# Thealexbarney/VGAudio

Hardware: NVIDIA H100
Metric: GC-ADPCM encode Msamples/sec (batch) (higher is better)
Workload: dtype int32

## Files before the change

vgaudio_b200/csrc/abi_gcadpcm.cu:

```cuda
#include <climits>

#include "abi.cuh"

using namespace vgb;

namespace {

struct GcLayout {
    int32_t n_channels = 0;
    std::vector<int64_t> pcm_off, adpcm_off, rec_off;
    std::vector<int32_t> n_samples, enc_count;
    std::vector<int16_t> hist;
    int64_t pcm_total = 0;
    int64_t adpcm_total = 0;
    int64_t rec_total = 0;
    int32_t max_frames = 0;
    int64_t total_frames = 0;
};

struct GcWorkspace {
    size_t off_pcm_off, off_adpcm_off, off_rec_off, off_n_samples, off_enc_count, off_hist, off_records, off_mask;
    size_t off_trace, off_used_start, off_stats;
    size_t off_status;
    size_t table_bytes;
    size_t total;
};

GcWorkspace carve(int64_t rec_total_frames, int32_t n_channels)
{
    GcWorkspace w{};
    size_t o = 0;
    auto take = [&](size_t bytes) { size_t at = o; o = align_up(o + bytes, 256); return at; };
    const size_t n = (size_t)(n_channels > 0 ? n_channels : 1);
    w.off_pcm_off = take(n * 8);
    w.off_adpcm_off = take(n * 8);
    w.off_rec_off = take(n * 8);
    w.off_n_samples = take(n * 4);
    w.off_enc_count = take(n * 4);
    w.off_hist = take(n * 4);
    w.table_bytes = o;
    w.off_records = take((size_t)rec_total_frames * sizeof(double2));
    w.off_mask = take((size_t)(rec_total_frames / 32 + 1) * 4);
    w.off_trace = take((size_t)rec_total_frames * 4);
    w.off_used_start = take(n * kGcMaxSegments * 4);
    w.off_stats = take(kGcStatWords * 8);
    w.off_status = take(16);
    w.total = o;
    return w;
}

int64_t padded_rec_bound(int64_t total_frames, int32_t n_channels) { return total_frames + 32ll * n_channels + 32; }

GcChannelTable table_view(void *ws, const GcWorkspace &w, int32_t n_channels)
{
    char *b = static_cast<char *>(ws);
    GcChannelTable t;
    t.pcm_off = reinterpret_cast<const int64_t *>(b + w.off_pcm_off);
    t.adpcm_off = reinterpret_cast<const int64_t *>(b + w.off_adpcm_off);
    t.rec_off = reinterpret_cast<const int64_t *>(b + w.off_rec_off);
    t.n_samples = reinterpret_cast<const int32_t *>(b + w.off_n_samples);
    t.enc_count = reinterpret_cast<const int32_t *>(b + w.off_enc_count);
    t.hist = reinterpret_cast<int16_t *>(b + w.off_hist);
    t.status = reinterpret_cast<int32_t *>(b + w.off_status);
    t.n_channels = n_channels;
    return t;
}

GcSegArgs seg_view(void *ws, const GcWorkspace &w, int32_t seg_count)
{
    char *b = static_cast<char *>(ws);
    GcSegArgs a;
    a.trace = reinterpret_cast<uint32_t *>(b + w.off_trace);
    a.used_start = reinterpret_cast<uint32_t *>(b + w.off_used_start);
    a.stats = reinterpret_cast<unsigned long long *>(b + w.off_stats);
    a.seg_count = seg_count;
    a.min_seg_frames = 0;
    return a;
}

int32_t upload_tables(const GcLayout &lay, const GcWorkspace &w, void *ws, cudaStream_t stream)
{
    std::vector<char> blob(w.table_bytes, 0);
    const size_t n = (size_t)lay.n_channels;
    if (n) {
        memcpy(blob.data() + w.off_pcm_off, lay.pcm_off.data(), n * 8);
        memcpy(blob.data() + w.off_adpcm_off, lay.adpcm_off.data(), n * 8);
        memcpy(blob.data() + w.off_rec_off, lay.rec_off.data(), n * 8);
        memcpy(blob.data() + w.off_n_samples, lay.n_samples.data(), n * 4);
        memcpy(blob.data() + w.off_enc_count, lay.enc_count.data(), n * 4);
        memcpy(blob.data() + w.off_hist, lay.hist.data(), n * 4);
    }
    CUDA_TRY(cudaMemcpyAsync(ws, blob.data(), w.table_bytes, cudaMemcpyHostToDevice, stream));
    return VGB_OK;
}

void layout_records(GcLayout &lay)
{
    lay.rec_off.resize(lay.n_channels);
    int64_t rec = 0;
    for (int c = 0; c < lay.n_channels; c++) {
        const int32_t frames = div_round_up(lay.n_samples[c], kGcFrameSamples);
        lay.rec_off[c] = rec;
        rec += (int64_t)align_up((size_t)frames, 32);
        if (frames > lay.max_frames) lay.max_frames = frames;
        lay.total_frames += div_round_up(lay.enc_count[c], kGcFrameSamples);
    }
    lay.rec_total = rec + 32;
}

int32_t layout_common(GcLayout &lay, const int32_t *n_samples, const vgb_gc_params *params, int32_t n_channels,
                      bool decode)
{
    if (n_channels < 0) return fail(VGB_E_ARG, "n_channels is negative (%d)", n_channels);
    if (n_channels > 0 && !n_samples) return fail(VGB_E_ARG, "n_samples is NULL");
    lay.n_channels = n_channels;
    lay.n_samples.resize(n_channels);
    lay.enc_count.resize(n_channels);
    lay.hist.assign((size_t)n_channels * 2, 0);
    for (int c = 0; c < n_channels; c++) {
        const int32_t n = n_samples[c];
        if (n < 0) return fail(VGB_E_ARG, "channel %d: negative sample count %d", c, n);
        int32_t enc = n;
        if (params) {
            if (!decode && params[c].sample_count != -1) {
                enc = params[c].sample_count;
                if (enc < 0 || enc > n)
                    return fail(VGB_E_ARG, "channel %d: sample_count %d outside the %d available samples", c, enc, n);
            }
            lay.hist[2 * c] = params[c].history1;
            lay.hist[2 * c + 1] = params[c].history2;
        }
        lay.n_samples[c] = n;
        lay.enc_count[c] = enc;
    }
    layout_records(lay);
    return VGB_OK;
}

void layout_pack_offsets(GcLayout &lay)
{
    lay.pcm_off.resize(lay.n_channels);
    lay.adpcm_off.resize(lay.n_channels);
    int64_t ps = 0, ab = 0;
    for (int c = 0; c < lay.n_channels; c++) {
        lay.pcm_off[c] = ps;
        lay.adpcm_off[c] = ab;
        ps += (int64_t)align_up((size_t)lay.n_samples[c], 8);
        ab += (int64_t)align_up((size_t)gc_sample_count_to_byte_count(lay.n_samples[c]), 16);
    }
    lay.pcm_total = ps + 8;
    lay.adpcm_total = ab + 16;
}

int max_encode_frames(const GcLayout &lay)
{
    int32_t m = 0;
    for (int c = 0; c < lay.n_channels; c++) m = std::max(m, div_round_up(lay.enc_count[c], kGcFrameSamples));
    return m;
}

int32_t run_gc_encode(const int16_t *d_pcm, const GcLayout &lay, const int16_t *d_coefs_in, int16_t *d_coefs_out,
                      uint8_t *d_adpcm, void *d_ws, const GcWorkspace &w, cudaStream_t stream, bool do_encode,
                      bool timed = true, bool tables_uploaded = false, cudaEvent_t after_coefs = nullptr)
{
    const bool was_timing = g_ctx.timing;
    if (!timed) g_ctx.timing = false;
    struct Restore { bool v; ~Restore() { g_ctx.timing = v; } } restore{was_timing};
    if (!tables_uploaded) VGB_TRY(upload_tables(lay, w, d_ws, stream));
    if (lay.n_channels == 0) return VGB_OK;
    GcChannelTable tab = table_view(d_ws, w, lay.n_channels);
    char *b = static_cast<char *>(d_ws);
    double2 *records = reinterpret_cast<double2 *>(b + w.off_records);
    uint32_t *mask = reinterpret_cast<uint32_t *>(b + w.off_mask);

    if (!d_coefs_in) {
        tick(0, true, stream);
        launch_gc_coef_frames(d_pcm, tab, records, mask, lay.max_frames, 0, INT_MAX, stream);
        tick(0, false, stream);
        tick(1, true, stream);
        launch_gc_coef_refine(tab, records, mask, d_coefs_out, stream);
        tick(1, false, stream);
        g_ctx.launches += (lay.max_frames > 0 ? 1 : 0) + 1;
    } else if (d_coefs_in != d_coefs_out) {
        CUDA_TRY(cudaMemcpyAsync(d_coefs_out, d_coefs_in, (size_t)lay.n_channels * 32, cudaMemcpyDeviceToDevice, stream));
    }
    if (after_coefs) CUDA_TRY(cudaEventRecord(after_coefs, stream));
    if (do_encode) {
        const int enc_frames = max_encode_frames(lay);
        int min_seg = 0;
        const int seg_count = gc_encode_pick_segments(lay.n_channels, enc_frames, &min_seg);
        GcSegArgs seg = seg_view(d_ws, w, seg_count);
        seg.min_seg_frames = min_seg;
        tick(2, true, stream);
        launch_gc_encode(d_pcm, tab, d_coefs_out, d_adpcm, lay.max_frames, 0, INT_MAX, seg, stream);
        tick(2, false, stream);
        g_ctx.launches += lay.max_frames > 0 ? (seg.seg_count > 1 ? 3 : 1) : 0;
        g_ctx.last_seg = seg;
    }
    CUDA_TRY(cudaGetLastError());
    return VGB_OK;
}

int32_t run_gc_decode(const uint8_t *d_adpcm, const GcLayout &lay, const int16_t *d_coefs, int16_t *d_pcm, void *d_ws,
                      const GcWorkspace &w, cudaStream_t stream)
{
    VGB_TRY(upload_tables(lay, w, d_ws, stream));
    if (lay.n_channels == 0) return VGB_OK;
    GcChannelTable tab = table_view(d_ws, w, lay.n_channels);
    CUDA_TRY(cudaMemsetAsync(tab.status, 0x7f, 4, stream));
    tick(3, true, stream);
    launch_gc_decode(d_adpcm, tab, d_coefs, d_pcm, lay.max_frames, 0, INT_MAX, stream);
    tick(3, false, stream);
    g_ctx.launches += lay.max_frames > 0 ? 1 : 0;
    CUDA_TRY(cudaGetLastError());
    return VGB_OK;
}


GcLayout sub_layout(const GcLayout &full, int c0, int c1)
{
    GcLayout g;
    g.n_channels = c1 - c0;
    g.pcm_off.assign(full.pcm_off.begin() + c0, full.pcm_off.begin() + c1);
    g.adpcm_off.assign(full.adpcm_off.begin() + c0, full.adpcm_off.begin() + c1);
    g.n_samples.assign(full.n_samples.begin() + c0, full.n_samples.begin() + c1);
    g.enc_count.assign(full.enc_count.begin() + c0, full.enc_count.begin() + c1);
    g.hist.assign(full.hist.begin() + 2 * c0, full.hist.begin() + 2 * c1);
    layout_records(g);
    return g;
}

int32_t host_encode_impl(const int16_t *const *pcm, const int32_t *n_samples, const vgb_gc_params *params,
                         const int16_t *coefs_in, int32_t n_channels, int16_t *coefs_out, uint8_t *const *adpcm_out,
                         vgb_progress_cb cb, void *user, bool do_encode)
{
    PinScope pins;
    GcLayout lay;
    VGB_TRY(layout_common(lay, n_samples, params, n_channels, false));
    if (n_channels == 0) return VGB_OK;
    if (!pcm) return fail(VGB_E_ARG, "pcm is NULL");
    if (!coefs_out) return fail(VGB_E_ARG, "coefs_out is NULL");
    if (do_encode && !adpcm_out) return fail(VGB_E_ARG, "adpcm_out is NULL");
    for (int c = 0; c < n_channels; c++) {
        if (!pcm[c] && lay.n_samples[c] > 0) return fail(VGB_E_ARG, "pcm[%d] is NULL", c);
        if (do_encode && !adpcm_out[c] && lay.enc_count[c] > 0) return fail(VGB_E_ARG, "adpcm_out[%d] is NULL", c);
    }
    layout_pack_offsets(lay);
    std::vector<int64_t> weight(n_channels), pcm_b(n_channels), pcm_len(n_channels), adpcm_len(n_channels);
    int64_t total = 0;
    for (int c = 0; c < n_channels; c++) {
        weight[c] = lay.n_samples[c];
        total += lay.n_samples[c];
        pcm_b[c] = lay.pcm_off[c] * 2;
        pcm_len[c] = (int64_t)lay.n_samples[c] * 2;
        adpcm_len[c] = gc_sample_count_to_byte_count(lay.enc_count[c]);
    }

    const int n_groups = pipeline_group_count(n_channels, 2 * total, 32, "VGB_ENCODE_GROUPS");
    const std::vector<int> bound = pipeline_bounds(weight, n_groups);

    std::lock_guard<std::mutex> lock(g_ctx.mu);
    VGB_TRY(ensure_ready_locked());
    std::vector<GcLayout> glay(n_groups);
    std::vector<GcWorkspace> gws(n_groups);
    std::vector<size_t> ws_at(n_groups);
    size_t ws_total = 0;
    for (int g = 0; g < n_groups; g++) {
        glay[g] = sub_layout(lay, bound[g], bound[g + 1]);
        gws[g] = carve(glay[g].rec_total, glay[g].n_channels);
        ws_at[g] = ws_total;
        ws_total += align_up(gws[g].total, 256);
    }
    VGB_TRY(g_ctx.pcm.reserve((size_t)lay.pcm_total * 2));
    VGB_TRY(g_ctx.adpcm.reserve((size_t)lay.adpcm_total));
    VGB_TRY(g_ctx.coefs.reserve((size_t)n_channels * 32 * 2));
    VGB_TRY(g_ctx.ws.reserve(ws_total));
    int16_t *d_coefs_out = static_cast<int16_t *>(g_ctx.coefs.p);
    int16_t *d_coefs_in = coefs_in ? d_coefs_out + (size_t)n_channels * 16 : nullptr;

    auto h2d = [&](int g) -> int32_t {
        const int c0 = bound[g], n = bound[g + 1] - c0;
        if (g == 0)
            for (int k = 0; k < n_groups; k++) VGB_TRY(upload_tables(glay[k], gws[k], g_ctx.ws.c() + ws_at[k], g_ctx.s_in));
        VGB_TRY(copy_units(cudaMemcpyHostToDevice, g_ctx.pcm.c(), pcm_b.data(), pcm, pcm_len.data(), c0, n, g_ctx.s_in));
        if (coefs_in && n > 0)
            CUDA_TRY(cudaMemcpyAsync(d_coefs_in + (size_t)c0 * 16, coefs_in + (size_t)c0 * 16, (size_t)n * 32,
                                     cudaMemcpyHostToDevice, g_ctx.s_in));
        return VGB_OK;
    };
    auto kern = [&](int g, cudaStream_t st, cudaEvent_t coefs_done) -> int32_t {
        const int c0 = bound[g];
        return run_gc_encode(static_cast<const int16_t *>(g_ctx.pcm.p), glay[g], d_coefs_in ? d_coefs_in + (size_t)c0 * 16 : nullptr,
                             d_coefs_out + (size_t)c0 * 16, static_cast<uint8_t *>(g_ctx.adpcm.p), g_ctx.ws.c() + ws_at[g], gws[g],
                             st, do_encode, false, true, coefs_done);
    };
    auto d2h = [&](int g) -> int32_t {
        const int c0 = bound[g], n = bound[g + 1] - c0;
        if (n > 0)
            CUDA_TRY(cudaMemcpyAsync(coefs_out + (size_t)c0 * 16, d_coefs_out + (size_t)c0 * 16, (size_t)n * 32,
                                     cudaMemcpyDeviceToHost, g_ctx.s_out));
        if (!do_encode) return VGB_OK;
        return copy_units(cudaMemcpyDeviceToHost, g_ctx.adpcm.c(), lay.adpcm_off.data(), adpcm_out, adpcm_len.data(), c0, n, g_ctx.s_out);
    };
    auto done = [&](int g) -> int32_t {
        if (cb && do_encode && glay[g].total_frames > 0) cb(user, glay[g].total_frames);
        return VGB_OK;
    };
    return run_group_pipeline(n_groups, h2d, kern, d2h, done);
}

int32_t host_encode_sharded(const int16_t *const *pcm, const int32_t *n_samples, const vgb_gc_params *params,
                            const int16_t *coefs_in, int32_t n_channels, int16_t *coefs_out, uint8_t *const *adpcm_out,
                            vgb_progress_cb cb, void *user, bool do_encode)
{
    if (!sharding_active(n_channels) || !pcm || !n_samples || !coefs_out || (do_encode && !adpcm_out))
        return host_encode_impl(pcm, n_samples, params, coefs_in, n_channels, coefs_out, adpcm_out, cb, user, do_encode);
    SharedProgress prog{cb, user, {}};
    return run_sharded(shard_units(n_channels, [&](int c) { return n_samples[c]; }, 64), [&](int, const std::vector<int> &u) -> int32_t {
        const int m = (int)u.size();
        auto s_pcm = pick_rows(pcm, u);
        auto s_n = pick_rows(n_samples, u);
        std::vector<vgb_gc_params> s_par;
        if (params) s_par = pick_rows(params, u);
        std::vector<int16_t> s_cin, s_cout((size_t)m * 16);
        if (coefs_in) s_cin = pick_rows(coefs_in, u, 16);
        std::vector<uint8_t *> s_out;
        if (do_encode) s_out = pick_rows(adpcm_out, u);
        VGB_TRY(host_encode_impl(s_pcm.data(), s_n.data(), params ? s_par.data() : nullptr, coefs_in ? s_cin.data() : nullptr, m,
                                 s_cout.data(), do_encode ? s_out.data() : nullptr, cb ? SharedProgress::relay : nullptr, &prog, do_encode));
        put_rows(coefs_out, u, s_cout, 16);
        return VGB_OK;
    });
}

}

extern "C" {

int32_t vgb_gcadpcm_sample_count_to_byte_count(int32_t n) { return gc_sample_count_to_byte_count(n); }
int32_t vgb_gcadpcm_byte_count_to_sample_count(int32_t b) { return gc_nibble_count_to_sample_count(b * 2); }
int32_t vgb_gcadpcm_sample_count_to_nibble_count(int32_t n) { return gc_sample_count_to_nibble_count(n); }
int32_t vgb_gcadpcm_nibble_count_to_sample_count(int32_t n) { return gc_nibble_count_to_sample_count(n); }
int32_t vgb_gcadpcm_sample_to_nibble(int32_t s)
{
    return kGcFrameNibbles * (s / kGcFrameSamples) + s % kGcFrameSamples + 2;
}
int32_t vgb_gcadpcm_nibble_to_sample(int32_t nib)
{
    return kGcFrameSamples * (nib / kGcFrameNibbles) + nib % kGcFrameNibbles - 2;
}

int32_t vgb_gcadpcm_coefs_batch(const int16_t *const *pcm, const int32_t *n_samples, int32_t n_channels,
                                int16_t *coefs_out)
{
    return host_encode_sharded(pcm, n_samples, nullptr, nullptr, n_channels, coefs_out, nullptr, nullptr, nullptr, false);
}

int32_t vgb_gcadpcm_encode_batch(const int16_t *const *pcm, const int32_t *n_samples, const vgb_gc_params *params,
                                 const int16_t *coefs_in, int32_t n_channels, int16_t *coefs_out,
                                 uint8_t *const *adpcm_out, vgb_progress_cb cb, void *user)
{
    return host_encode_sharded(pcm, n_samples, params, coefs_in, n_channels, coefs_out, adpcm_out, cb, user, true);
}

static int32_t gcadpcm_decode_one(const uint8_t *const *adpcm, const int32_t *n_bytes, const int16_t *coefs,
                                  const vgb_gc_params *params, int32_t n_channels, int16_t *const *pcm_out)
{
    PinScope pins;
    if (n_channels < 0) return fail(VGB_E_ARG, "n_channels is negative (%d)", n_channels);
    if (n_channels == 0) return VGB_OK;
    if (!adpcm || !n_bytes || !coefs || !pcm_out) return fail(VGB_E_ARG, "NULL argument");
    std::vector<int32_t> counts(n_channels);
    for (int c = 0; c < n_channels; c++) {
        if (n_bytes[c] < 0) return fail(VGB_E_ARG, "channel %d: negative byte count", c);
        int32_t want = (params && params[c].sample_count != -1) ? params[c].sample_count
                                                                : gc_nibble_count_to_sample_count(n_bytes[c] * 2);
        if (want < 0) return fail(VGB_E_ARG, "channel %d: negative sample count %d", c, want);
// ... 407 lines not shown
```

vgaudio_b200/csrc/common.cuh:

```cuda
#pragma once

#include <cuda_runtime.h>
#include <stdint.h>

namespace vgb {

constexpr int kGcFrameSamples = 14;
constexpr int kGcFrameBytes = 8;
constexpr int kGcFrameNibbles = 16;

__host__ __device__ __forceinline__ int32_t wadd(int32_t a, int32_t b) { return (int32_t)((uint32_t)a + (uint32_t)b); }
__host__ __device__ __forceinline__ int32_t wsub(int32_t a, int32_t b) { return (int32_t)((uint32_t)a - (uint32_t)b); }
__host__ __device__ __forceinline__ int32_t wmul(int32_t a, int32_t b) { return (int32_t)((uint32_t)a * (uint32_t)b); }

__host__ __device__ __forceinline__ int32_t clamp16(int32_t v) { return v > 32767 ? 32767 : (v < -32768 ? -32768 : v); }
__host__ __device__ __forceinline__ int32_t clamp4(int32_t v) { return v > 7 ? 7 : (v < -8 ? -8 : v); }

__host__ __device__ __forceinline__ int32_t gc_sample_count_to_nibble_count(int32_t n)
{
    int32_t whole = n / kGcFrameSamples, rest = n % kGcFrameSamples;
    return kGcFrameNibbles * whole + (rest == 0 ? 0 : rest + 2);
}
__host__ __device__ __forceinline__ int32_t gc_sample_count_to_byte_count(int32_t n)
{
    int32_t nib = gc_sample_count_to_nibble_count(n);
    return nib / 2 + (nib & 1);
}
__host__ __device__ __forceinline__ int32_t gc_nibble_count_to_sample_count(int32_t nib)
{
    int32_t whole = nib / kGcFrameNibbles, rest = nib % kGcFrameNibbles;
    return kGcFrameSamples * whole + (rest < 2 ? 0 : rest - 2);
}
__host__ __device__ __forceinline__ int32_t div_round_up(int32_t a, int32_t b) { return (int32_t)(((int64_t)a + b - 1) / b); }

struct GcChannelTable {
    const int64_t *pcm_off;
    const int64_t *adpcm_off;
    const int64_t *rec_off;
    const int32_t *n_samples;
    const int32_t *enc_count;
    int16_t *hist;
    int32_t *status;
    int32_t n_channels;
};

constexpr int kGcMinSegFrames = 4096;
constexpr int kGcMaxSegments = 256;
constexpr int kGcStatWords = 18;
struct GcSegArgs {
    uint32_t *trace;
    uint32_t *used_start;
    unsigned long long *stats;
    int32_t seg_count;
    int32_t min_seg_frames;
};

struct GcTapChannel {
    int64_t out_off;
    int32_t samples_per_entry;
    int32_t loop_start;
};

struct AdxChannel {
    int64_t pcm_off;
    int64_t adpcm_off;
    int32_t n_samples;
    int32_t frame_size, version, padding, type, filter;
    int32_t history;
    int16_t coef0, coef1;
    int64_t trace_off;
};

constexpr int kAdxMinSegFrames = 4096;
constexpr int kAdxMaxSegments = 64;
struct AdxSegArgs {
    uint32_t *trace;
    uint32_t *used_start;
    unsigned long long *stats;
    int32_t seg_count;
    int32_t min_seg_frames;
};

constexpr int32_t VGB_HCA_BITRATE_TOO_LOW = 1;
constexpr int32_t VGB_HCA_NOT_IMPLEMENTED = 2;
constexpr int32_t VGB_HCA_BIT_OVERFLOW = 3;
constexpr int32_t VGB_HCA_BAD_SYNC = 4;
constexpr int32_t VGB_HCA_BAD_INDEX = 6;
constexpr int32_t VGB_HCA_BAD_DELTA = 5;

struct HcaConfig {
    int32_t channel_count, frame_size;
    int32_t base_band_count, stereo_band_count, total_band_count, hfr_band_count, bands_per_hfr_group, hfr_group_count;
    int32_t channel_type[8];
    uint8_t ath[128];
};

struct HcaStream {
    int64_t pcm_off;
    int64_t channel_stride;
    int64_t frames_off;
    int64_t dct_off;
    int32_t sample_count, frame_count;
    int32_t inserted_samples, reserved;
    int32_t pre_zero, pre_fill, post_count, loop_start, src_count, last_chunk;
};

struct HcaTables {
    const double *window;
    const double *sin_tab[8], *cos_tab[8];
    const int32_t *shuffle;
    double mdct_scale, sqrt2;
    const double *dequantizer_scaling, *quantizer_scaling;
    const double *inv_step, *dead_zone;
    const double *intensity_bounds;
    const uint8_t *scale_to_resolution;
    const uint8_t *quantized_max_bits;
    const uint8_t (*quantize_bits)[16];
    const uint8_t (*quantize_value)[16];
    const uint16_t *crc_table;
    const double *step_size;
    const double *intensity_ratio;
    const double *scale_conversion;
    const uint8_t (*dequantize_bits)[16];
    const int8_t (*dequantize_value)[16];
};

}
```

vgaudio_b200/csrc/gc_encode.cu:

```cuda
#include <algorithm>
#include <cstdlib>

#include "common.cuh"
#include "kernels.h"

namespace vgb {

constexpr uint32_t kFull = 0xFFFFFFFFu;
constexpr int kEncChunkFrames = 16;
constexpr int kEncChunkSamples = kEncChunkFrames * kGcFrameSamples;
constexpr int kEncWarps = 2;
constexpr int kEncWarpChannels = 4;
constexpr int kEncRowPad = 4;
#ifndef VGB_ENC_BLOCKS_PER_SM
#define VGB_ENC_BLOCKS_PER_SM 8
#endif
constexpr int kEncChainBlocksPerSm = VGB_ENC_BLOCKS_PER_SM;
constexpr uint32_t kErrSat = (1u << 27) - 1;

template <bool kGeneral>
struct GcTrial {
    uint32_t w0, w1;
    int32_t r1, r2;
    int32_t over;
    uint64_t err;
    int32_t recon[kGeneral ? 14 : 1];
};

__device__ __forceinline__ int32_t gc_quantise_exact(int32_t diff, int shift)
{
    const uint32_t a = diff < 0 ? (0u - (uint32_t)diff) : (uint32_t)diff;
    const uint32_t top = a >> 24;
    const uint32_t hs = top ? (0x80000000u >> __clz(top)) : 0u;
    const uint32_t m = (a + (1u << (shift - 1)) - 1u - hs) >> shift;
    return diff < 0 ? -(int32_t)m : (int32_t)m;
}

template <bool kGeneral>
__device__ __forceinline__ void gc_attempt_exact(const int16_t *frame, int n, int32_t h1, int32_t h2, int32_t c0,
                                              int32_t c1, int sp, GcTrial<kGeneral> &t)
{
    const int shift = sp + 11;
    const int32_t scale = (int32_t)(1u << shift);
    int32_t r1 = h1, r2 = h2, over = 0;
    uint64_t err = 0;
    uint32_t w0 = 0, w1 = 0;
#pragma unroll
    for (int s = 0; s < 14; s++) {
        if (kGeneral && s >= n) break;
        const int32_t xs = frame[s];
        const int32_t want = xs * 2048;
        const int32_t guess = wadd(wmul(r2, c1), wmul(r1, c0));
        const int32_t diff = wsub(want, guess);
        const int32_t raw = gc_quantise_exact(diff, shift);
        const int32_t q = clamp4(raw);
        over = max(over, abs(raw - q));
        const int32_t out = clamp16(wadd(wadd(guess, wmul(q, scale)), 1024) >> 11);
        const int32_t miss = xs - out;
        err += (uint64_t)((int64_t)miss * miss);
        const int byte = 1 + s / 2, bit = (byte & 3) * 8 + ((s & 1) ? 0 : 4);
        if (byte < 4) w0 |= (uint32_t)(q & 15) << bit; else w1 |= (uint32_t)(q & 15) << bit;
        if (kGeneral) t.recon[s] = out;
        r2 = r1;
        r1 = out;
    }
    t.w0 = w0; t.w1 = w1; t.r1 = r1; t.r2 = r2; t.over = over; t.err = err;
}

__device__ __forceinline__ int32_t imad(int32_t a, int32_t b, int32_t c)
{
    int32_t d;
    asm("mad.lo.s32 %0, %1, %2, %3;" : "=r"(d) : "r"(a), "r"(b), "r"(c));
    return d;
}

__device__ __forceinline__ int32_t sar(int32_t a, int k)
{
    int32_t d;
    asm("shr.s32 %0, %1, %2;" : "=r"(d) : "r"(a), "r"(k));
    return d;
}

template <bool kGeneral>
__device__ __forceinline__ void gc_try_predictor_literal(const int16_t *frame, int n, int32_t h1, int32_t h2, int32_t c0,
                                                         int32_t c1, int sp_first, GcTrial<kGeneral> &t, int &sp_out)
{
    int sp = sp_first - 1;
    do {
        sp++;
        gc_attempt_exact<kGeneral>(frame, n, h1, h2, c0, c1, sp, t);
        const int pass_power = sp;
        for (int v = t.over + 8; v > 256; v >>= 1)
            if (++sp >= 12) sp = 11;
        if (pass_power >= 12) { sp = 12; break; }
    } while (sp < 12 && t.over > 1);
    sp_out = sp;
}

__device__ __forceinline__ uint32_t gc_peak_key(int32_t older, int32_t newer, int32_t cur, int32_t c0, int32_t c1, int s,
                                                int32_t neg_bias = 0)
{
    const int32_t guess = imad(newer, c0, imad(older, c1, neg_bias)) / 2048;
    const int32_t diff = clamp16(wsub(cur, guess));
    return ((uint32_t)abs(diff) << 5) | ((uint32_t)(15 - s) << 1) | ((uint32_t)diff >> 31);
}

__device__ __forceinline__ void gc_peak_terms(int32_t older, int32_t newer, int32_t cur, int32_t c0, int32_t c1, int s,
                                              int32_t neg_bias, int32_t &tp, int32_t &tn)
{
    const int32_t g = imad(newer, c0, imad(older, c1, neg_bias));
    const int32_t q = (int32_t)(g + (int32_t)((uint32_t)(g >> 31) >> 21)) >> 11;
    const int32_t d = imad(q, -1, cur);
    tp = imad(d, 16, 15 - s - 32768 * 16);
    tn = imad(d, -16, 15 - s + 32768 * 16);
}
__device__ __forceinline__ uint32_t gc_peak_pack(int32_t kp, int32_t kn)
{
    const int32_t k = max(kp, kn);
    return ((uint32_t)k << 1) | (uint32_t)(kn > kp);
}
constexpr uint32_t kPeakKeyMax = (32768u << 5) | 1u;

__device__ __forceinline__ int gc_first_scale_power(uint32_t key)
{
    int top;
    asm("bfind.u32 %0, %1;" : "=r"(top) : "r"(key));
    const int n = max(top - 7, 0);
    const uint32_t t = key >> ((n + 4) & 31);
    const uint32_t one_less = ((t - 9u) >> 31) & key & ((uint32_t)(-n) >> 31);
    return max(n - 1 - (int)one_less, 0);
}

__device__ __forceinline__ uint32_t quarter_min_u32(uint32_t v)
{
    v = min(v, __shfl_xor_sync(kFull, v, 1));
    v = min(v, __shfl_xor_sync(kFull, v, 2));
    return min(v, __shfl_xor_sync(kFull, v, 4));
}

__device__ __noinline__ uint32_t gc_slow_frame(const int16_t *frame, int32_t h1, int32_t h2, int32_t c0, int32_t c1,
                                               int sp_first, int lane, bool commit, uint8_t *out8)
{
    const int pred = lane & 7;
    GcTrial<false> t;
    t.err = 0; t.r1 = 0; t.r2 = 0; t.w0 = 0; t.w1 = 0;
    int sp_final = 0;
    gc_try_predictor_literal<false>(frame, 14, h1, h2, c0, c1, sp_first, t, sp_final);
    const uint64_t full_key = (t.err << 3) | (uint64_t)pred;
    const uint32_t hi = (uint32_t)(full_key >> 16);
    const uint32_t min_hi = quarter_min_u32(hi);
    const uint32_t lo = hi == min_hi ? (uint32_t)(full_key & 0xFFFFu) : 0xFFFFFFFFu;
    const uint32_t min_lo = quarter_min_u32(lo);
    if (hi == min_hi && lo == min_lo && commit) {
        const uint32_t head = (uint32_t)((pred << 4) | (sp_final & 0xF));
        *reinterpret_cast<uint2 *>(out8) = make_uint2(t.w0 | head, t.w1);
    }
    const uint32_t mine = (uint32_t)(t.r1 + 32768) | ((uint32_t)(t.r2 + 32768) << 16);
    return __shfl_sync(kFull, mine, (lane & ~7) | (int)(min_lo & 7u));
}

struct GcPass {
    int sp;
    bool valid;
    int shift;
    int32_t mul;
    int32_t base_g;
    int32_t base_t;
    uint32_t near_c;
    uint32_t near_k;
    int32_t lmul;
    int32_t r1, r2;
    int32_t rmin, rmax, raw_even;
    uint32_t nearmin;
    uint32_t near_even;
    uint32_t nw0, nw1;
    uint64_t e0, e1;
};

__device__ __forceinline__ void gc_pass_begin(GcPass &P, int sp_raw, int32_t bias_c, int32_t p1, int32_t p2)
{
    P.sp = min(sp_raw, 12);
    P.valid = sp_raw <= 12;
    P.shift = P.sp + 11;
    P.mul = (int32_t)(1u << P.sp);
    P.base_g = wsub(wsub(1024, (int32_t)(8u << P.shift)), bias_c);
    P.base_t = wadd(P.base_g, wadd(bias_c, (int32_t)(1u << (P.shift - 1))) - 1 - 32768 * 2048);
    const int lsh = 32 - P.shift;
    P.near_c = 128u << lsh;
    P.near_k = (1u << lsh) + P.near_c;
    P.lmul = (int32_t)(1u << lsh);
    P.r1 = p1; P.r2 = p2;
    P.rmin = 0; P.rmax = 0; P.raw_even = 0;
    P.nearmin = 0xFFFFFFFFu;
    P.near_even = 0xFFFFFFFFu;
    P.nw0 = 0; P.nw1 = 0;
    P.e0 = 0; P.e1 = 0;
}

__device__ __forceinline__ void gc_pass_step(GcPass &P, int s, int32_t xs, int32_t xw, int32_t c0, int32_t c1)
{
    const int32_t gn = imad(P.r2, c1, P.base_g);
    const int32_t wf = imad(P.r1, c0, gn);
    const int32_t tm1 = wsub(wadd(xw, P.base_t), wf);
    const int32_t t2 = tm1 + (int32_t)((uint32_t)tm1 >> 31);
    const int32_t raw = sar(t2, P.shift);
    const int32_t qb = __viaddmin_s32_relu(raw, 8, 15);
    const int32_t o = imad(qb, P.mul, wf >> 11);
    const int32_t ob = __viaddmin_s32_relu(o, 32768, 65535);
    P.r2 = P.r1;
    P.r1 = ob;
    if (s & 1) {
        P.rmin = __vimin3_s32(P.rmin, P.raw_even, raw);
        P.rmax = __vimax3_s32(P.rmax, P.raw_even, raw);
    } else {
        P.raw_even = raw;
    }
    const uint32_t near = (uint32_t)imad(tm1, P.lmul, (int32_t)P.near_k);
    if (s & 1) P.nearmin = __vimin3_u32(P.nearmin, P.near_even, near);
    else P.near_even = near;
    const int32_t miss = imad(ob, -1, xs);
    const uint64_t sq = (uint64_t)((int64_t)miss * miss);
    if (s & 1) P.e1 += sq; else P.e0 += sq;
    const int byte = 1 + s / 2, bit = (byte & 3) * 8 + ((s & 1) ? 0 : 4);
    if (byte < 4) P.nw0 = (uint32_t)imad(qb, 1 << bit, (int32_t)P.nw0);
    else P.nw1 = (uint32_t)imad(qb, (int32_t)(1u << bit), (int32_t)P.nw1);
}

__device__ __forceinline__ void gc_pass_end(const GcPass &P, bool &term, bool &trouble)
{
    const int32_t m = __viaddmax_s32(P.rmax, 1, -P.rmin);
    const int32_t m_scaled = imad(m, P.mul, 0);
    const bool big = m_scaled >= (1 << 13);
    const bool huge = m_scaled >= (1 << 18);
    const bool over_ge_240 = m >= 248;
    const bool over_gt_248 = m >= 257;
    const bool over_le_1 = m <= 9;
    const bool near = (P.nearmin <= 2u * P.near_c) | over_ge_240;
    trouble = P.valid & ((huge | (big & near)) | ((P.sp < 12) & over_gt_248));
    term = P.valid & (over_le_1 | (P.sp >= 12));
}

constexpr int kGcChain = 0, kGcRunOn = 1, kGcCascade = 2;

__host__ __device__ __forceinline__ int gc_seg_len(int range_frames, int seg_count, int min_seg_frames)
{
    const int per = (div_round_up(range_frames, seg_count > 0 ? seg_count : 1) + kEncChunkFrames - 1) / kEncChunkFrames * kEncChunkFrames;
    return per < min_seg_frames ? min_seg_frames : per;
}

template <int kMode>
__global__ void __launch_bounds__(kEncWarps * 32, kMode == kGcChain ? kEncChainBlocksPerSm : 1)
gc_encode_kernel(const int16_t *__restrict__ pcm, GcChannelTable tab, const int16_t *__restrict__ coefs,
                 uint8_t *__restrict__ adpcm, int frame_begin, int frame_end, GcSegArgs sa)
{
    __shared__ __align__(16) int16_t in_buf[kEncWarps][kEncWarpChannels][2][kEncChunkSamples];
    __shared__ __align__(16) int32_t x_buf[kEncWarps][kEncWarpChannels][2 * kEncChunkSamples + kEncRowPad];
    __shared__ __align__(16) uint8_t out_buf[kEncWarps][kEncWarpChannels][kEncChunkFrames * kGcFrameBytes];

    const int warp = threadIdx.x >> 5, lane = threadIdx.x & 31;
    const int qc = lane >> 3, pred = lane & 7;
    const int ch0 = (blockIdx.x * kEncWarps + warp) * kEncWarpChannels;
    if (ch0 >= tab.n_channels) return;
    const bool live = ch0 + qc < tab.n_channels;
    const int ch = live ? ch0 + qc : tab.n_channels - 1;

    const int n_enc = live ? tab.enc_count[ch] : 0;
    const int n_frames = div_round_up(n_enc, kGcFrameSamples);
    const int f_end = min(frame_end, n_frames);
    const int range_frames = max(f_end - frame_begin, 0);
    const int seg_len = gc_seg_len(range_frames, sa.seg_count, sa.min_seg_frames);
    const int total_bytes = gc_sample_count_to_byte_count(n_enc);

    const int16_t *src = pcm + tab.pcm_off[ch];
    uint8_t *dst = adpcm + tab.adpcm_off[ch];
    uint32_t *trace = sa.trace + tab.rec_off[ch];
    uint32_t *used_start = sa.used_start + (int64_t)ch * sa.seg_count;
    const int32_t c0 = coefs[(int64_t)ch * 16 + 2 * pred];
    const int32_t c1 = coefs[(int64_t)ch * 16 + 2 * pred + 1];
    const int32_t bias_c = wmul(32768, wadd(c0, c1));
    int16_t (*const in_row)[kEncChunkSamples] = in_buf[warp][qc];
    int32_t *const x_row = x_buf[warp][qc];

    auto stage_chunk = [&](int chunk_frame, int b) {
#pragma unroll
        for (int k = 0; k < 4; k++) {
            const int v = pred + 8 * k;
            if (v < kEncChunkSamples / 8) {
                const int64_t s = (int64_t)chunk_frame * kGcFrameSamples + v * 8;
                int64_t valid = (int64_t)n_enc - s;
                valid = valid < 0 ? 0 : (valid > 8 ? 8 : valid);
                const int16_t *from = valid > 0 ? src + s : src;
                const unsigned to = (unsigned)__cvta_generic_to_shared(&in_row[b][v * 8]);
                asm volatile("cp.async.cg.shared.global [%0], [%1], 16, %2;" ::"r"(to), "l"(from), "r"((int)valid * 2) : "memory");
            }
        }
        asm volatile("cp.async.commit_group;" ::: "memory");
    };
    auto staged_wait = [&]() {
        asm volatile("cp.async.wait_group 0;" ::: "memory");
        __syncwarp();
    };
    auto widen_chunk = [&](int b) {
#pragma unroll
        for (int h = 0; h < 2; h++) {
            const int f = pred + 8 * h;
            const uint32_t *from = reinterpret_cast<const uint32_t *>(&in_row[b][f * kGcFrameSamples]);
            int2 *to = reinterpret_cast<int2 *>(&x_row[b * kEncChunkSamples + f * kGcFrameSamples]);
#pragma unroll
            for (int k = 0; k < kGcFrameSamples / 2; k++) {
                const uint32_t w = from[k];
                to[k] = make_int2((int32_t)(int16_t)(w & 0xFFFFu) + 32768, ((int32_t)w >> 16) + 32768);
            }
        }
        __syncwarp();
    };
    auto key_rest_of = [&](const int32_t *frame) -> uint32_t {
        int32_t v[14];
#pragma unroll
        for (int j = 0; j < 14; j++) v[j] = frame[j];
        int32_t kp = 0, kn = 0;
#pragma unroll
        for (int j = 2; j < 14; j += 2) {
            int32_t tpa, tna, tpb, tnb;
            gc_peak_terms(v[j - 2], v[j - 1], v[j], c0, c1, j, -bias_c, tpa, tna);
            gc_peak_terms(v[j - 1], v[j], v[j + 1], c0, c1, j + 1, -bias_c, tpb, tnb);
            kp = __vimax3_s32(kp, tpa, tpb);
            kn = __vimax3_s32(kn, tna, tnb);
        }
        return gc_peak_pack(kp, kn);
    };

    const int job_first = kMode == kGcChain ? (int)blockIdx.y : (kMode == kGcRunOn ? (int)blockIdx.y + 1 : 1);
    const int job_last = kMode == kGcCascade ? sa.seg_count - 1 : job_first;
    int truth_upto = 0;
    int reencoded = 0;
    int32_t p1 = 0, p2 = 0;

    for (int job = job_first; job <= job_last; job++) {
        const int seg_lo = frame_begin + job * seg_len;
        bool need = live && seg_lo < f_end;
        uint32_t start_pair = 0;
        if (kMode == kGcChain) {
            if (need) {
                if (job == 0) {
                    p1 = tab.hist[2 * ch] + 32768; p2 = tab.hist[2 * ch + 1] + 32768;
                } else {
                    p1 = src[(int64_t)seg_lo * kGcFrameSamples - 1] + 32768; p2 = src[(int64_t)seg_lo * kGcFrameSamples - 2] + 32768;
                }
            }
        } else {
            if (kMode == kGcCascade) __syncwarp();
            if (need) start_pair = trace[seg_lo - 1];
            if (kMode == kGcRunOn) {
                if (need && pred == 0) used_start[job] = start_pair;
            } else {
                need = need && seg_lo >= truth_upto && start_pair != used_start[job];
            }
            p1 = (int32_t)(start_pair & 0xFFFFu); p2 = (int32_t)(start_pair >> 16);
        }
        const int seg_hi = kMode == kGcCascade ? f_end : min(seg_lo + seg_len, f_end);
        const int len = need ? seg_hi - seg_lo : 0;
        int len_warp = max(len, __shfl_xor_sync(kFull, len, 8));
        len_warp = max(len_warp, __shfl_xor_sync(kFull, len_warp, 16));
        if (len_warp == 0) continue;
        bool spliced = false;
        int done = 0;

    int buf = 0;
    stage_chunk(seg_lo, 0);
    staged_wait();
    widen_chunk(0);
    uint32_t key_rest = key_rest_of(x_row);

    for (int rc = 0; rc < len_warp; rc += kEncChunkFrames) {
        const int cf = seg_lo + rc;
        stage_chunk(cf + kEncChunkFrames, buf ^ 1);
        const int frames_warp = min(kEncChunkFrames, len_warp - rc);
        const int frames_here = max(min(kEncChunkFrames, len - rc), 0);
        const int32_t *chunk = x_row + buf * kEncChunkSamples;
        const int32_t *other = x_row + (buf ^ 1) * kEncChunkSamples;
        uint32_t tr0 = 0, tr1 = 0;
        uint32_t tr_old0 = 0, tr_old1 = 0;
        if (kMode != kGcChain && !spliced) {
            if (pred < frames_here) tr_old0 = trace[cf + pred];
            if (pred + 8 < frames_here) tr_old1 = trace[cf + pred + 8];
        }
        int frames_done = 0;
        bool all_done = false;

        for (int i = 0; i < frames_warp; i++) {
            if (i == kEncChunkFrames - 1) {
                staged_wait();
                widen_chunk(buf ^ 1);
            }
            const bool active = i < frames_here && !spliced;
            const int32_t *frame = chunk + i * kGcFrameSamples;
            const int32_t *frame_next = (i + 1 < kEncChunkFrames) ? frame + kGcFrameSamples : other;
            int32_t x[14];
#pragma unroll
            for (int j = 0; j < 14; j++) x[j] = frame[j];

            int32_t tp0, tn0, tp1, tn1;
            gc_peak_terms(p2, p1, x[0], c0, c1, 0, -bias_c, tp0, tn0);
            gc_peak_terms(p1, x[0], x[1], c0, c1, 1, -bias_c, tp1, tn1);
            const uint32_t key = min(max(key_rest, gc_peak_pack(max(tp0, tp1), max(tn0, tn1))), kPeakKeyMax);
            const int sp_first = gc_first_scale_power(key);

            uint32_t w0 = 0, w1 = 0;
            uint64_t err = 0;
            int sp = 0;
            int32_t q1 = p1, q2 = p2;
            uint32_t key_rest_next = 0;
            bool resolved = !active;
            bool trouble = false;

#pragma unroll
            for (int round = 0; round < 2; round++) {
                GcPass A, B;
                gc_pass_begin(A, sp_first + 2 * round, bias_c, p1, p2);
                if (round == 0) gc_pass_begin(B, sp_first + 1, bias_c, p1, p2);
#pragma unroll
                for (int s = 0; s < 14; s++) {
                    const int32_t xw = imad(x[s], 2048, 0);
                    gc_pass_step(A, s, x[s], xw, c0, c1);
                    if (round == 0) gc_pass_step(B, s, x[s], xw, c0, c1);
                    if (round == 0 && s == 4) key_rest_next = key_rest_of(frame_next);
                }
                bool term_a, trouble_a, term_b = false, trouble_b = false;
                gc_pass_end(A, term_a, trouble_a);
                if (round == 0) gc_pass_end(B, term_b, trouble_b);
                const bool take = round == 0 || !resolved;
                const bool use_b = round == 0 && !term_a;
                if (take) {
                    trouble = trouble | (active & (trouble_a | (use_b & trouble_b)));
                    err = use_b ? B.e0 + B.e1 : A.e0 + A.e1;
                    w0 = (use_b ? B.nw0 : A.nw0) ^ 0x88888800u;
                    w1 = (use_b ? B.nw1 : A.nw1) ^ 0x88888888u;
                    sp = use_b ? B.sp : A.sp;
                    q1 = use_b ? B.r1 : A.r1;
                    q2 = use_b ? B.r2 : A.r2;
                    resolved = resolved | term_a | term_b;
                }
                if (round == 0 && !__any_sync(kFull, !resolved)) break;
            }
            trouble = trouble | !resolved;

            const uint32_t e_sat = err < (uint64_t)kErrSat ? (uint32_t)err : kErrSat;
            uint32_t best = quarter_min_u32(active ? ((e_sat << 3) | (uint32_t)pred) : 0xFFFFFFFFu);
            const bool sat = (best >> 3) >= kErrSat && best != 0xFFFFFFFFu;
            if (__any_sync(kFull, sat)) {
                const uint64_t full_key = active ? ((err << 3) | (uint64_t)pred) : ~0ull;
                const uint32_t hi = (uint32_t)(full_key >> 16);
                const uint32_t min_hi = quarter_min_u32(hi);
                best = quarter_min_u32(hi == min_hi ? (uint32_t)(full_key & 0xFFFFu) : 0xFFFFFFFFu);
            }
            const int best_lane = (lane & ~7) | (int)(best & 7u);
            const uint32_t head = (uint32_t)((pred << 4) | sp);
            uint8_t *out8 = &out_buf[warp][qc][i * kGcFrameBytes];
            if (lane == best_lane && active) *reinterpret_cast<uint2 *>(out8) = make_uint2(w0 | head, w1);
            uint32_t packed = __shfl_sync(kFull, (uint32_t)q1 | ((uint32_t)q2 << 16), best_lane);
            const uint32_t trouble_bits = __ballot_sync(kFull, trouble);
            if (trouble_bits != 0u) {
                __syncwarp();
                const bool mine = ((trouble_bits >> (lane & ~7)) & 0xFFu) != 0u && active;
                const uint32_t redo = gc_slow_frame(&in_row[buf][i * kGcFrameSamples], p1 - 32768, p2 - 32768, c0, c1, sp_first, lane, mine, out8);
                if (mine) packed = redo;
            }
            if (active) {
                p1 = (int32_t)(packed & 0xFFFFu);
                p2 = (int32_t)(packed >> 16);
                frames_done = i + 1;
                if (pred == i) tr0 = packed;
                if (pred + 8 == i) tr1 = packed;
            }
            if (kMode != kGcChain) {
                const uint32_t old = __shfl_sync(kFull, i < 8 ? tr_old0 : tr_old1, (lane & ~7) | (i & 7));
                if (active && packed == old) spliced = true;
                all_done = __all_sync(kFull, spliced || rc + i + 1 >= len);
                if (all_done) break;
            }

            key_rest = key_rest_next;
        }
        staged_wait();

        if (frames_done > 0) {
            const int64_t byte0 = (int64_t)cf * kGcFrameBytes;
            const int bytes_here = (int)min((int64_t)frames_done * kGcFrameBytes, (int64_t)total_bytes - byte0);
            const int b = pred * 16;
            if (b + 16 <= bytes_here) {
                *reinterpret_cast<uint4 *>(dst + byte0 + b) = *reinterpret_cast<const uint4 *>(&out_buf[warp][qc][b]);
            } else {
                for (int j = b; j < bytes_here; j++) dst[byte0 + j] = out_buf[warp][qc][j];
            }
            if (pred < frames_done) trace[cf + pred] = tr0;
            if (pred + 8 < frames_done) trace[cf + pred + 8] = tr1;
            done += frames_done;
        }
        __syncwarp();
        buf ^= 1;
        if (kMode != kGcChain && all_done) break;
    }
        if (kMode != kGcChain) {
            reencoded += done;
            if (kMode == kGcCascade && need) truth_upto = seg_lo + done;
            if (kMode == kGcRunOn && need && !spliced && pred == 0 && seg_hi < f_end)
                atomicAdd(&sa.stats[2], 1ull);
            if (kMode == kGcRunOn && need && pred == 0) {
                atomicMax(&sa.stats[3], (unsigned long long)done);
                atomicAdd(&sa.stats[4 + min(31 - __clz(max(done, 1)), 13)], 1ull);
            }
        }
    }

    if (kMode != kGcChain && pred == 0 && reencoded > 0) atomicAdd(&sa.stats[kMode == kGcRunOn ? 0 : 1], (unsigned long long)reencoded);
    if ((kMode == kGcCascade || (kMode == kGcChain && sa.seg_count == 1)) && live && range_frames > 0) {
        __syncwarp();
        if (pred == 0) {
            const uint32_t last = trace[f_end - 1];
            tab.hist[2 * ch] = (int16_t)((int32_t)(last & 0xFFFFu) - 32768);
            tab.hist[2 * ch + 1] = (int16_t)((int32_t)(last >> 16) - 32768);
        }
    }
}

__global__ void __launch_bounds__(128)
gc_encode_frames_kernel(int16_t *__restrict__ pcm_in_out, const int32_t *__restrict__ sample_count,
                        const int16_t *__restrict__ coefs, int n_frames, uint8_t *__restrict__ adpcm_out)
{
    __shared__ int16_t stage[4][16];
    const int lane = threadIdx.x & 31, warp = threadIdx.x >> 5;
    const int f = blockIdx.x * (blockDim.x >> 5) + warp;
    if (f >= n_frames) return;
    int16_t *io = pcm_in_out + (int64_t)f * 16;
    const int n = sample_count ? min(max(sample_count[f], 0), 14) : 14;
    if (lane < 16) stage[warp][lane] = io[lane];
    __syncwarp();
    const int16_t *frame = &stage[warp][2];
    const int32_t h2 = stage[warp][0], h1 = stage[warp][1];
    const int pred = lane >> 2, cand = lane & 3;
    const int32_t c0 = coefs[(int64_t)f * 16 + 2 * pred], c1 = coefs[(int64_t)f * 16 + 2 * pred + 1];

    uint32_t key = 0;
#pragma unroll
    for (int s = 0; s < 14; s++) {
        if (s >= n) break;
        const int32_t older = s == 0 ? h2 : (s == 1 ? h1 : (int32_t)frame[s >= 2 ? s - 2 : 0]);
        const int32_t newer = s == 0 ? h1 : (int32_t)frame[s >= 1 ? s - 1 : 0];
        key = max(key, gc_peak_key(older, newer, frame[s], c0, c1, s));
    }
    const int sp_first = gc_first_scale_power(key);

    GcTrial<true> t;
    t.err = 0;
    int sp_final = 0;
    const bool pred_winner = cand == 0;
    if (pred_winner) gc_try_predictor_literal<true>(frame, n, h1, h2, c0, c1, sp_first, t, sp_final);
    const uint64_t full_key = pred_winner ? ((t.err << 5) | (uint64_t)lane) : ~0ull;
    const uint32_t hi = (uint32_t)(full_key >> 16);
    const uint32_t min_hi = __reduce_min_sync(kFull, hi);
    const uint32_t lo = (pred_winner && hi == min_hi) ? (uint32_t)(full_key & 0xFFFFu) : 0xFFFFFFFFu;
    const uint32_t min_lo = __reduce_min_sync(kFull, lo);
    const bool is_winner = pred_winner && hi == min_hi && lo == min_lo;
    if (is_winner) {
        const uint32_t head = (uint32_t)((pred << 4) | (sp_final & 0xF));
        uint32_t w[2] = {t.w0 | head, t.w1};
        for (int j = 0; j < 8; j++) adpcm_out[(int64_t)f * 8 + j] = (uint8_t)(w[j >> 2] >> ((j & 3) * 8));
#pragma unroll
        for (int j = 0; j < 14; j++)
            if (j < n) io[2 + j] = (int16_t)t.recon[j];
    }
}

int gc_encode_min_segment_frames()
{
    if (const char *env = std::getenv("VGB_GC_MIN_SEG_FRAMES")) {
        const int v = std::atoi(env);
        if (v >= kEncChunkFrames) return (v + kEncChunkFrames - 1) / kEncChunkFrames * kEncChunkFrames;
    }
    return kGcMinSegFrames;
}

int gc_encode_pick_segments(int n_channels, int max_frames, int *min_seg_out)
{
    int min_seg = gc_encode_min_segment_frames();
    if (min_seg_out) *min_seg_out = min_seg;
    if (const char *env = std::getenv("VGB_GC_SEGMENTS")) {
        const int v = std::atoi(env);
        if (v >= 1) return v > kGcMaxSegments ? kGcMaxSegments : v;
    }
    static int slots = 0;
    if (slots == 0) {
        int dev = 0, sms = 132, per_sm = kEncChainBlocksPerSm;
        cudaGetDevice(&dev);
        cudaDeviceGetAttribute(&sms, cudaDevAttrMultiProcessorCount, dev);
        if (cudaOccupancyMaxActiveBlocksPerMultiprocessor(&per_sm, gc_encode_kernel<kGcChain>, kEncWarps * 32, 0) != cudaSuccess || per_sm < 1) {
            (void)cudaGetLastError();
            per_sm = kEncChainBlocksPerSm;
        }
        slots = sms * per_sm * kEncWarps;
    }
    const int rows = (n_channels + kEncWarpChannels - 1) / kEncWarpChannels;
    const int five_waves = (int)((5ll * slots + rows - 1) / rows);
    if (!std::getenv("VGB_GC_MIN_SEG_FRAMES") && max_frames / min_seg < std::min(five_waves, 8)) min_seg = std::max(kEncChunkFrames, min_seg / 2);
    if (min_seg_out) *min_seg_out = min_seg;
    const int max_s = std::min(kGcMaxSegments, std::max(1, max_frames / min_seg));
    int best = 1;
    long long best_cost = -1;
    for (int s = 1; s <= max_s; s++) {
        const long long waves = ((long long)rows * s + slots - 1) / slots;
        const long long cost = waves * gc_seg_len(max_frames, s, min_seg);
        if (best_cost < 0 || cost <= best_cost) { best = s; best_cost = cost; }
    }
    return best;
}

void launch_gc_encode(const int16_t *pcm, const GcChannelTable &tab, const int16_t *coefs, uint8_t *adpcm,
                      int max_frames, int frame_begin, int frame_end, GcSegArgs sa, cudaStream_t stream)
{
    if (tab.n_channels <= 0 || max_frames <= 0) return;
    if (frame_begin >= frame_end || frame_begin >= max_frames) return;
    const int per_block = kEncWarps * kEncWarpChannels;
    const int blocks = (tab.n_channels + per_block - 1) / per_block;
    if (sa.seg_count < 1) sa.seg_count = 1;
    if (sa.seg_count > kGcMaxSegments) sa.seg_count = kGcMaxSegments;
    if (sa.min_seg_frames <= 0) sa.min_seg_frames = gc_encode_min_segment_frames();
    cudaMemsetAsync(sa.stats, 0, kGcStatWords * sizeof(unsigned long long), stream);
    gc_encode_kernel<kGcChain><<<dim3(blocks, sa.seg_count), kEncWarps * 32, 0, stream>>>(pcm, tab, coefs, adpcm, frame_begin, frame_end, sa);
    if (sa.seg_count > 1) {
        gc_encode_kernel<kGcRunOn><<<dim3(blocks, sa.seg_count - 1), kEncWarps * 32, 0, stream>>>(pcm, tab, coefs, adpcm, frame_begin, frame_end, sa);
        gc_encode_kernel<kGcCascade><<<dim3(blocks, 1), kEncWarps * 32, 0, stream>>>(pcm, tab, coefs, adpcm, frame_begin, frame_end, sa);
    }
}

void launch_gc_encode_frames(int16_t *pcm_in_out, const int32_t *sample_count, const int16_t *coefs, int n_frames,
                             uint8_t *adpcm_out, cudaStream_t stream)
{
    if (n_frames <= 0) return;
    int blocks = (n_frames + 3) / 4;
    gc_encode_frames_kernel<<<blocks, 128, 0, stream>>>(pcm_in_out, sample_count, coefs, n_frames, adpcm_out);
}

}
```

Before: 29600.

## Overlap run-on pass with chain pass via programmatic launch and per-segment flags

Adds per-row, per-segment completion flags that the chain kernel sets with release stores. When the grid is large relative to resident capacity, the run-on kernel is launched with programmatic stream serialization so it can start early, and each warp spin-waits with acquire loads until its two neighbouring chain segments are done. Trace reads switch to L2-only loads so the early consumer sees fresh data. This aims to hide the tail and launch gap between the two kernels, at the cost of spin-waiting and a possible deadlock risk if waiting blocks occupy slots that chain blocks still need.

```diff
diff --git a/vgaudio_b200/csrc/abi_gcadpcm.cu b/vgaudio_b200/csrc/abi_gcadpcm.cu
--- a/vgaudio_b200/csrc/abi_gcadpcm.cu
+++ b/vgaudio_b200/csrc/abi_gcadpcm.cu
@@ -43,7 +43,7 @@
     w.off_mask = take((size_t)(rec_total_frames / 32 + 1) * 4);
     w.off_trace = take((size_t)rec_total_frames * 4);
     w.off_used_start = take(n * kGcMaxSegments * 4);
-    w.off_stats = take(kGcStatWords * 8);
+    w.off_stats = take(kGcStatWords * 8 + gc_seg_done_words((int32_t)n) * 4);
     w.off_status = take(16);
     w.total = o;
     return w;
@@ -73,6 +73,7 @@
     a.trace = reinterpret_cast<uint32_t *>(b + w.off_trace);
     a.used_start = reinterpret_cast<uint32_t *>(b + w.off_used_start);
     a.stats = reinterpret_cast<unsigned long long *>(b + w.off_stats);
+    a.seg_done = reinterpret_cast<uint32_t *>(a.stats + kGcStatWords);
     a.seg_count = seg_count;
     a.min_seg_frames = 0;
     return a;
diff --git a/vgaudio_b200/csrc/common.cuh b/vgaudio_b200/csrc/common.cuh
--- a/vgaudio_b200/csrc/common.cuh
+++ b/vgaudio_b200/csrc/common.cuh
@@ -47,10 +47,15 @@
 constexpr int kGcMinSegFrames = 4096;
 constexpr int kGcMaxSegments = 256;
 constexpr int kGcStatWords = 18;
+__host__ __device__ __forceinline__ size_t gc_seg_done_words(int32_t n_channels)
+{
+    return ((size_t)(n_channels > 0 ? n_channels : 1) / 4 + 2) * (size_t)kGcMaxSegments;
+}
 struct GcSegArgs {
     uint32_t *trace;
     uint32_t *used_start;
     unsigned long long *stats;
+    uint32_t *seg_done;
     int32_t seg_count;
     int32_t min_seg_frames;
 };
diff --git a/vgaudio_b200/csrc/gc_encode.cu b/vgaudio_b200/csrc/gc_encode.cu
--- a/vgaudio_b200/csrc/gc_encode.cu
+++ b/vgaudio_b200/csrc/gc_encode.cu
@@ -67,6 +67,17 @@
     t.w0 = w0; t.w1 = w1; t.r1 = r1; t.r2 = r2; t.over = over; t.err = err;
 }
 
+__device__ __forceinline__ uint32_t ld_acquire_u32(const uint32_t *p)
+{
+    uint32_t v;
+    asm volatile("ld.acquire.gpu.global.u32 %0, [%1];" : "=r"(v) : "l"(p) : "memory");
+    return v;
+}
+__device__ __forceinline__ void st_release_u32(uint32_t *p, uint32_t v)
+{
+    asm volatile("st.release.gpu.global.u32 [%0], %1;" ::"l"(p), "r"(v) : "memory");
+}
+
 __device__ __forceinline__ int32_t imad(int32_t a, int32_t b, int32_t c)
 {
     int32_t d;
@@ -259,7 +270,9 @@
 
     const int warp = threadIdx.x >> 5, lane = threadIdx.x & 31;
     const int qc = lane >> 3, pred = lane & 7;
-    const int ch0 = (blockIdx.x * kEncWarps + warp) * kEncWarpChannels;
+    if (kMode == kGcChain) asm volatile("griddepcontrol.launch_dependents;" ::: "memory");
+    const int row = blockIdx.x * kEncWarps + warp;
+    const int ch0 = row * kEncWarpChannels;
     if (ch0 >= tab.n_channels) return;
     const bool live = ch0 + qc < tab.n_channels;
     const int ch = live ? ch0 + qc : tab.n_channels - 1;
@@ -278,6 +291,13 @@
     const int32_t c0 = coefs[(int64_t)ch * 16 + 2 * pred];
     const int32_t c1 = coefs[(int64_t)ch * 16 + 2 * pred + 1];
     const int32_t bias_c = wmul(32768, wadd(c0, c1));
+    if (kMode == kGcRunOn) {
+        if (lane == 0) {
+            const uint32_t *done = sa.seg_done + (int64_t)row * sa.seg_count + blockIdx.y;
+            while (ld_acquire_u32(done) == 0u || ld_acquire_u32(done + 1) == 0u) __nanosleep(2000);
+        }
+        __syncwarp();
+    }
     int16_t (*const in_row)[kEncChunkSamples] = in_buf[warp][qc];
     int32_t *const x_row = x_buf[warp][qc];
 
@@ -350,7 +370,7 @@
             }
         } else {
             if (kMode == kGcCascade) __syncwarp();
-            if (need) start_pair = trace[seg_lo - 1];
+            if (need) start_pair = __ldcg(&trace[seg_lo - 1]);
             if (kMode == kGcRunOn) {
                 if (need && pred == 0) used_start[job] = start_pair;
             } else {
@@ -382,8 +402,8 @@
         uint32_t tr0 = 0, tr1 = 0;
         uint32_t tr_old0 = 0, tr_old1 = 0;
         if (kMode != kGcChain && !spliced) {
-            if (pred < frames_here) tr_old0 = trace[cf + pred];
-            if (pred + 8 < frames_here) tr_old1 = trace[cf + pred + 8];
+            if (pred < frames_here) tr_old0 = __ldcg(&trace[cf + pred]);
+            if (pred + 8 < frames_here) tr_old1 = __ldcg(&trace[cf + pred + 8]);
         }
         int frames_done = 0;
         bool all_done = false;
@@ -513,6 +533,13 @@
         }
     }
 
+    if (kMode == kGcChain && sa.seg_count > 1) {
+        __syncwarp();
+        if (lane == 0) {
+            __threadfence();
+            st_release_u32(sa.seg_done + (int64_t)row * sa.seg_count + blockIdx.y, 1u);
+        }
+    }
     if (kMode != kGcChain && pred == 0 && reencoded > 0) atomicAdd(&sa.stats[kMode == kGcRunOn ? 0 : 1], (unsigned long long)reencoded);
     if ((kMode == kGcCascade || (kMode == kGcChain && sa.seg_count == 1)) && live && range_frames > 0) {
         __syncwarp();
@@ -581,16 +608,10 @@
     return kGcMinSegFrames;
 }
 
-int gc_encode_pick_segments(int n_channels, int max_frames, int *min_seg_out)
-{
-    int min_seg = gc_encode_min_segment_frames();
-    if (min_seg_out) *min_seg_out = min_seg;
-    if (const char *env = std::getenv("VGB_GC_SEGMENTS")) {
-        const int v = std::atoi(env);
-        if (v >= 1) return v > kGcMaxSegments ? kGcMaxSegments : v;
-    }
-    static int slots = 0;
-    if (slots == 0) {
+static int gc_encode_chain_resident_blocks()
+{
+    static int blocks = 0;
+    if (blocks == 0) {
         int dev = 0, sms = 132, per_sm = kEncChainBlocksPerSm;
         cudaGetDevice(&dev);
         cudaDeviceGetAttribute(&sms, cudaDevAttrMultiProcessorCount, dev);
@@ -598,8 +619,20 @@
             (void)cudaGetLastError();
             per_sm = kEncChainBlocksPerSm;
         }
-        slots = sms * per_sm * kEncWarps;
-    }
+        blocks = sms * per_sm;
+    }
+    return blocks;
+}
+
+int gc_encode_pick_segments(int n_channels, int max_frames, int *min_seg_out)
+{
+    int min_seg = gc_encode_min_segment_frames();
+    if (min_seg_out) *min_seg_out = min_seg;
+    if (const char *env = std::getenv("VGB_GC_SEGMENTS")) {
+        const int v = std::atoi(env);
+        if (v >= 1) return v > kGcMaxSegments ? kGcMaxSegments : v;
+    }
+    const int slots = gc_encode_chain_resident_blocks() * kEncWarps;
     const int rows = (n_channels + kEncWarpChannels - 1) / kEncWarpChannels;
     const int five_waves = (int)((5ll * slots + rows - 1) / rows);
     if (!std::getenv("VGB_GC_MIN_SEG_FRAMES") && max_frames / min_seg < std::min(five_waves, 8)) min_seg = std::max(kEncChunkFrames, min_seg / 2);
@@ -625,10 +658,20 @@
     if (sa.seg_count < 1) sa.seg_count = 1;
     if (sa.seg_count > kGcMaxSegments) sa.seg_count = kGcMaxSegments;
     if (sa.min_seg_frames <= 0) sa.min_seg_frames = gc_encode_min_segment_frames();
-    cudaMemsetAsync(sa.stats, 0, kGcStatWords * sizeof(unsigned long long), stream);
+    cudaMemsetAsync(sa.stats, 0, kGcStatWords * sizeof(unsigned long long) + (size_t)blocks * kEncWarps * sa.seg_count * 4, stream);
     gc_encode_kernel<kGcChain><<<dim3(blocks, sa.seg_count), kEncWarps * 32, 0, stream>>>(pcm, tab, coefs, adpcm, frame_begin, frame_end, sa);
     if (sa.seg_count > 1) {
-        gc_encode_kernel<kGcRunOn><<<dim3(blocks, sa.seg_count - 1), kEncWarps * 32, 0, stream>>>(pcm, tab, coefs, adpcm, frame_begin, frame_end, sa);
+        const bool early = (long long)blocks * sa.seg_count >= 2ll * gc_encode_chain_resident_blocks();
+        cudaLaunchConfig_t cfg = {};
+        cfg.gridDim = dim3(blocks, sa.seg_count - 1);
+        cfg.blockDim = dim3(kEncWarps * 32);
+        cfg.stream = stream;
+        cudaLaunchAttribute attr[1];
+        attr[0].id = cudaLaunchAttributeProgrammaticStreamSerialization;
+        attr[0].val.programmaticStreamSerializationAllowed = 1;
+        cfg.attrs = attr;
+        cfg.numAttrs = early ? 1 : 0;
+        cudaLaunchKernelEx(&cfg, gc_encode_kernel<kGcRunOn>, pcm, tab, coefs, adpcm, frame_begin, frame_end, sa);
         gc_encode_kernel<kGcCascade><<<dim3(blocks, 1), kEncWarps * 32, 0, stream>>>(pcm, tab, coefs, adpcm, frame_begin, frame_end, sa);
     }
 }
```

Measured after the change: 29730, median of 6. About the same (+0.5%).
